# mir-group/allegro

Hardware: AMD Instinct MI355X
Metric: edge tensor-products/sec (forward+force) (higher is better)
Workload: dtype f32; 1 GPU; c4: bulk Si 23^3 cells (97 336 atoms), r_cut 5 A, l_max=2, L=2, u=64; atoms=97336, edges=2725408, parallelism=single GPU, weights=random init (reference initialisers), seed 456, workspace_bytes=21849491824

## Files before the change

### allegro_amd/_lib.py

```python
import ctypes as C
import os
from typing import Optional

import numpy as np

AA_MAX_LAYERS = 4
AA_MAX_MLP_LAYERS = 4
AA_F32, AA_F64 = 0, 1

_dp = C.POINTER(C.c_double)
_ip = C.POINTER(C.c_int32)


class TpDesc(C.Structure):
    _fields_ = [("mul", C.c_int32), ("d1", C.c_int32), ("d2", C.c_int32), ("dout", C.c_int32),
                ("num_paths", C.c_int32), ("coupling", C.c_int32), ("nnz", C.c_int32),
                ("nz_i", _ip), ("nz_j", _ip), ("nz_k", _ip), ("nz_path", _ip), ("nz_val", _dp)]


class ModelConfig(C.Structure):
    _fields_ = [("dtype", C.c_int32), ("num_types", C.c_int32), ("num_bessels", C.c_int32), ("poly_p", C.c_double),
                ("l_max", C.c_int32), ("num_layers", C.c_int32), ("num_scalar", C.c_int32), ("num_tensor", C.c_int32),
                ("embed_dim", C.c_int32), ("embed_mlp_depth", C.c_int32), ("embed_mlp_width", C.c_int32),
                ("latent_mlp_depth", C.c_int32), ("latent_mlp_width", C.c_int32),
# ... 12 lines not shown


def options_from_env() -> PlanOptions:
    env = os.environ
    flag = lambda k: int(env.get(k, "0")[:1] == "1")
    o = PlanOptions()
    o.tp_generic, o.tp_no_chain, o.tp_no_moments = flag("AA_TP_GENERIC"), flag("AA_TP_NOCHAIN"), flag("AA_TP_NOMOM")
    o.tp_no_operator, o.tp_force_operator, o.tp_operator_fused = flag("AA_TP_NOOP"), flag("AA_TP_OP"), flag("AA_OP_NOSPLIT")
    o.gemm_no_chain, o.gemm_fp32_mfma, o.gemm_valu, o.gemm_v1 = (flag("AA_GEMM_NOCHAIN"), flag("AA_GEMM_FP32_MFMA"),
                                                                 flag("AA_GEMM_VALU"), flag("AA_GEMM_V1"))
    o.gemm_lds_epilogue = int(env.get("AA_GEMM_DIRECT_EPILOGUE", "1")[:1] == "0")
    o.f64_column_loop = {"0": 1, "2": 2}.get(env.get("AA_F64_NLOOP", "1")[:1], 0)
    o.embed_no_fuse = flag("AA_EMBED_NOFUSE")
    o.fused_forward = {"0": 3, "1": 1, "2": 2, "4": 4}.get(env.get("AA_FUSED", "")[:1], 0)
    o.moments_waves_per_block = int(env.get("AA_MOM_WPB", "0") or 0)
    o.no_channel_padding = flag("AA_NO_PAD")
    o.no_slot_form = flag("AA_NO_SLOT_FORM")
    o.op_proj_gemm = {"1": 1, "0": 2}.get(env.get("AA_OP_PROJ", "")[:1], 0)
    o.op_env_vector = flag("AA_OP_ENV_VECTOR")
    o.staged_no_fold = flag("AA_STAGED_NOFOLD")
    o.op_recompute_bvecs = flag("AA_OP_RECOMPUTE_BVECS")
    o.readout_two_pass = flag("AA_READOUT_TWO_PASS")
    o.tp_prefer_moments = flag("AA_TP_PREFER_MOM")
    o.fused_narrow = {"1": 1, "2": 2, "3": 3}.get(env.get("AA_FUSED_NARROW", "")[:1], 0)
    o.chain_staged_weights = flag("AA_CHAIN_STAGED")
    o.poison_workspace = flag("AA_POISON")
    o.f64_rows = {"0": 2, "2": 1}.get(env.get("AA_F64_ROWS", "")[:1], 0)
    return o


class RawWeights(C.Structure):
    _fields_ = [("rmax_recip", _dp), ("bessel_weights", _dp), ("center_embed", _dp), ("neighbor_embed", _dp),
                ("basis_linear", _dp), ("embed_mlp", _dp * AA_MAX_MLP_LAYERS), ("env_embed_linear", _dp),
                ("first_proj", _dp), ("latent", (_dp * AA_MAX_MLP_LAYERS) * AA_MAX_LAYERS),
                ("tp_weights", _dp * AA_MAX_LAYERS), ("readout", _dp * AA_MAX_MLP_LAYERS), ("scales", _dp),
                ("shifts", _dp), ("spline_weights", _dp)]


class Graph(C.Structure):
    _fields_ = [("num_atoms", C.c_int64), ("num_edges", C.c_int64), ("center", C.c_void_p), ("nbr", C.c_void_p),
                ("rowptr", C.c_void_p), ("types", C.c_void_p), ("shift_vec", C.c_void_p),
                ("t_rowptr", C.c_void_p), ("t_perm", C.c_void_p), ("atom_begin", C.c_int64), ("atom_end", C.c_int64),
                ("max_degree", C.c_int64)]


class GemmSeg(C.Structure):
    _fields_ = [("p", C.c_void_p), ("ld", C.c_int32), ("n", C.c_int32)]
# ... 218 lines not shown
```

### allegro_amd/csrc/aa_common.h

```cpp
#pragma once
#include <type_traits>
#include <hip/hip_runtime.h>

#include <algorithm>
#include <cmath>
#include <cstdint>
#include <cstdio>
#include <cstring>
#include <string>
#include <vector>

#include "allegro_amd.h"

extern __shared__ unsigned char aa_smem[];

namespace aa {

void set_error(const std::string& msg);
int fail(int code, const std::string& msg);
int device_cu_count();

#define AA_CHECK_HIP(expr)                                                                      \
  do {                                                                                          \
    hipError_t _e = (expr);                                                                     \
// ... 538 lines not shown
  int coupling;
  float sf;
  const float* ro_w;
  float ro_factor;
  const float *scales, *shifts;
  float* vec;
  float* sh;
  float* se_h;
  float* emb;
  float* w0;
  float* lat_h0;
  float* lat_h1;
  float* ro_h;
  float* fcat;
  float *x2s0, *x2s1;
  float* atom_energy;
  int long_only;
  int32_t* status;
  int mixed;
  int skip_long, fill_done;
  float* g_fcat;
  float* g_scal1;
  int ld_gfcat;
};
size_t fused_fwd_lds_bytes(int num_types, bool teams);
enum class FusedForm { OneWave, FourWave, EightWave, EightWaveTail };
int fused_fwd_num_steps(int R);
int launch_fused_fwd(int pair, FusedForm form, const FusedFwdArgs& a, const FusedFwdArgs* wide, hipStream_t stream);
int fused_fwd8_num_steps(int R, bool tail);
size_t fused_fwd8_lds_bytes(int num_types, int waves);
int launch_fused_fwd8(int pair, FusedForm form, const FusedFwdArgs& a, hipStream_t stream);


struct EdgeGeomArgs {
  int64_t E, N;
  const int32_t *center, *nbr, *types;
  const void* pos;
  const void* shift_vec;
  int num_types, num_bessels, l_max, S0;
  double poly_p;
  const void* rmax_recip;
  const void* bessel_w;
  const void* center_embed;
  const void* neighbor_embed;
  const void* basis_w;
  int embed_kind, spline_span;
  const void* emb_tab;
  void* vec;
  void* sh;
  void* emb0;
};
template <typename T>
// ... 56 lines not shown
```

### allegro_amd/csrc/aa_fused8.hip

```cpp
#include "aa_fused_tile.h"

namespace aa {

#ifdef AA_FUSED_TIMING
__device__ unsigned long long g_fused8_ticks[32];
#define AA_TICK8(i) \
  if (blockIdx.x == gridDim.x / 2 && threadIdx.x == 0) g_fused8_ticks[i] = __builtin_readcyclecounter();
#else
#define AA_TICK8(i)
#endif

namespace {

constexpr int kLdY8 = 12;
constexpr int kOffB8 = 32 * kLdT;
constexpr int kOffY8 = kOffB8 + 9 * 64;
constexpr int kOffPark8 = kOffY8 + 32 * kLdY8;
constexpr int fused_wave_floats(int waves) { return kOffPark8 + (waves == 8 ? 2 : 1) * kTileFloats; }
static_assert(64 * kLdY8 <= 32 * kLdT, "sM must fit the patch");

template <int D>
__device__ __forceinline__ void tile_moments_half(float* sT, const float* sY, const v16f& t0, const v16f& t1, int lane, float* M) {
  const int el = lane & 31, hh = lane >> 5;
  float M0[D], M1[D];
#pragma unroll
  for (int j = 0; j < D; ++j) {
    M0[j] = 0.f;
    M1[j] = 0.f;
  }
  auto pass = [&](const v16f& t, float* Mx) {
    __builtin_amdgcn_wave_barrier();
#pragma unroll
    for (int q = 0; q < 4; ++q) *reinterpret_cast<v4f*>(sT + el * kLdT + 8 * q + 4 * hh) = v4f{t[4 * q], t[4 * q + 1], t[4 * q + 2], t[4 * q + 3]};
    __builtin_amdgcn_wave_barrier();
    const float* col = sT + (16 * hh) * kLdT + el;
    const float* yr = sY + (16 * hh) * kLdY8;
#pragma unroll 4
    for (int i = 0; i < 16; ++i) {
      const float a = col[i * kLdT];
      float y[12];
#pragma unroll
      for (int q = 0; q < (D + 3) / 4; ++q) {
        const v4f yy = *reinterpret_cast<const v4f*>(yr + i * kLdY8 + 4 * q);
#pragma unroll
        for (int c = 0; c < 4; ++c) y[4 * q + c] = yy[c];
      }
#pragma unroll
      for (int j = 0; j < D; ++j) Mx[j] += y[j] * a;
    }
    __builtin_amdgcn_wave_barrier();
  };
  pass(t0, M0);
  pass(t1, M1);
#pragma unroll
  for (int j = 0; j < D; ++j) {
    permlane32_swap(M0[j], M1[j]);
    M[j] = M0[j] + M1[j];
  }
}

template <int S, int NS, class Args, class Pipe, class F>
__device__ __forceinline__ void fused_step8(const Args& A, Pipe& p, const XSplit& x, v16f& a0, v16f& a1, F&& between) {
  pipe_issue<S, NS>(A, p);
  fused_mma_step(p.wbuf + (S & 1) * kWStep, p.lane, x, a0, a1);
  between();
  pipe_commit<S>(p);
}


__device__ __forceinline__ v16f tile_load_rows8(const float* base, unsigned ld, int lane, bool row_ok) {
  unsigned el = lane & 31;
  const unsigned hh = lane >> 5;
  opaque_vector(el);
  v16f t;
  const unsigned off = (el * ld + 4u * hh) * 4u;
#pragma unroll
  for (int q = 0; q < 4; ++q) {
    v4f v = {0.f, 0.f, 0.f, 0.f};
    if (row_ok) v = *reinterpret_cast<const v4f*>(at_bytes(base, off + 32u * q));
#pragma unroll
    for (int i = 0; i < 4; ++i) t[4 * q + i] = v[i];
// ... 38 lines not shown
    for (int i = 0; i < 4; ++i) {
      if (g < 4)
        s0[4 * q + i] += w0a[4 * q + i] * T4[i];
      else
        s1[4 * q + i] += w0b[4 * q + i] * T4[i];
    }
    if (g < 4)
      anchor(s0);
    else
      anchor(s1);
    __builtin_amdgcn_sched_barrier(0);
  }
}

struct TileIn8 {
  int beg, cnt;
  int j;
  float pi[3], pj[3], sv[3];
  int ti, tj;
};

}

constexpr int fused_fwd8_steps(int R, bool tail) { return 4 + (2 + 2 * R) + 4 + 4 + 2 + 8 + 2 + (tail ? 12 : 0); }

template <class Sig0, class Sig1, int WAVES, bool TAIL>
__global__ __launch_bounds__(64 * WAVES, 2) void fused_fwd8_kernel(FusedFwdArgs A) {
  static_assert(WAVES == 8 || WAVES == 4, "workgroup forms");
  constexpr int NT = 64 * WAVES;
  constexpr int NPARK = WAVES == 8 ? 2 : 1;
  constexpr int kWaveF = kOffPark8 + NPARK * kTileFloats;
  constexpr int D = Sig0::D2, R = Sig0::LMAX + 1;
  static_assert(Sig0::D1 == D && Sig0::DOUT == D && Sig1::D1 == D && Sig1::DOUT == 1, "standard 2-layer stack");
  static_assert(D <= 9, "l_max <= 2");
  constexpr int kPS = 4;
  constexpr int S_P0 = 0, S_L2 = kPS, S_L3 = S_L2 + 2 + 2 * R, S_P1 = S_L3 + 4, S_L6A = S_P1 + kPS, S_M = S_L6A + 2, S_L8K = S_M + 8, S_T = S_L8K + 2,
                NS = S_T + (TAIL ? 12 : 0);
  static_assert(NS % 2 == 0 && NS <= kFusedMaxSteps && NS == fused_fwd8_steps(R, TAIL), "program length");
  u32x4* wbuf = reinterpret_cast<u32x4*>(aa_smem);
  float* sRo = reinterpret_cast<float*>(wbuf + 2 * kWStep);
  float* sRm = sRo + 64;
  float* sTab = sRm + 32;
  const int ntab = A.num_types * A.num_types * 512;
  const int tid = threadIdx.x, lane = tid & 63, hh = lane >> 5, el = lane & 31;
  const int wvs = __builtin_amdgcn_readfirstlane(tid >> 6);
  float* sW = sTab + ntab + wvs * kWaveF;
  float* sBv = sW + kOffB8;
  float* sY = sW + kOffY8;
  float* sPark = sW + kOffPark8;
  for (int i = tid; i < 64; i += NT) sRo[i] = A.ro_w[i];
  if (tid < A.num_types * A.num_types) sRm[tid] = A.rmax_recip[tid];
  if (tid >= 16 && tid < 24) sRm[tid] = A.embed_kind == 0 ? A.bessel_w[tid - 16] : 0.f;
  for (int i = tid; i < ntab; i += NT) sTab[i] = A.emb_tab[i];
  std::conditional_t<WAVES == 8, FusedPipe8, FusedPipe> p;
  p.wbuf = wbuf;
  p.tid = tid;
  p.lane = lane;
  p.zero = 0;
  if constexpr (WAVES == 8) {
    p.wv = wvs;
// ... 276 lines not shown
    for (int r = 0; r < 16; ++r) {
      a60[r] = 0.f;
      a61[r] = 0.f;
      a80[r] = 0.f;
      a81[r] = 0.f;
    }
    {
      XSplit xs[2];
      v16f t;
      xsplit_from_acc(sc0, xs[0]);
      fused_step8<S_L6A + 0, NS>(A, p, xs[0], a60, a61, [&] { xsplit_from_acc(sc1, xs[1]); });
      fused_step8<S_L6A + 1, NS>(A, p, xs[1], a60, a61, [&] { xsplit_from_acc(k0, xs[0]); });
      fused_step8<S_M + 0, NS>(A, p, xs[0], a60, a61, [&] {});
      fused_step8<S_M + 1, NS>(A, p, xs[0], a80, a81, [&] { xsplit_from_acc(k1, xs[1]); });
      fused_step8<S_M + 2, NS>(A, p, xs[1], a60, a61, [&] { t = fetch_tile(sPark, lane); });
      fused_step8<S_M + 3, NS>(A, p, xs[1], a80, a81, [&] { xsplit_from_acc(t, xs[0]); });
      fused_step8<S_M + 4, NS>(A, p, xs[0], a60, a61, [&] {
        if constexpr (NPARK == 2) t = fetch_tile(sPark + kTileFloats, lane); else t = tbr;
      });
      fused_step8<S_M + 5, NS>(A, p, xs[0], a80, a81, [&] { xsplit_from_acc(t, xs[1]); });
      fused_step8<S_M + 6, NS>(A, p, xs[1], a60, a61, [&] {});
      fused_step8<S_M + 7, NS>(A, p, xs[1], a80, a81, [&] {});
      AA_TICK8(8)
      if constexpr (TAIL) {
#pragma unroll
        for (int r = 0; r < 16; ++r) {
          dk0[r] = dsilu(a60[r]);
          dk1[r] = dsilu(a61[r]);
        }
      } else {
        tile_store_rows8(sW, a60, (A.lat_h1) + row0 * 64, cnt, 64, lane);
        tile_store_rows8(sW, a61, (A.lat_h1 + 32) + row0 * 64, cnt, 64, lane);
      }
      keep_tile<true>(a60, k0);
      keep_tile<true>(a61, k1);
      xsplit_from_acc(k0, xs[0]);
      fused_step8<S_L8K + 0, NS>(A, p, xs[0], a80, a81, [&] { xsplit_from_acc(k1, xs[1]); });
      fused_step8<S_L8K + 1, NS>(A, p, xs[1], a80, a81, [&] {});
    }
    AA_TICK8(9)
    {
      if constexpr (!TAIL) {
        tile_store_rows8(sW, a80, (A.ro_h) + row0 * 64, cnt, 64, lane);
        tile_store_rows8(sW, a81, (A.ro_h + 32) + row0 * 64, cnt, 64, lane);
      }
      float part = 0.f;
#pragma unroll
      for (int q = 0; q < 4; ++q) {
        const v4f w0v = *reinterpret_cast<const v4f*>(sRo + 8 * q + 4 * hh);
        const v4f w1v = *reinterpret_cast<const v4f*>(sRo + 32 + 8 * q + 4 * hh);
#pragma unroll
        for (int i = 0; i < 4; ++i) part += silu(a80[4 * q + i]) * w0v[i] + silu(a81[4 * q + i]) * w1v[i];
      }
      float tot = row_ok ? part : 0.f;
#pragma unroll
      for (int m = 32; m >= 1; m >>= 1) tot += __shfl_xor(tot, m);
      if (atom_ok && lane == 0) {
        float en = tot * A.ro_factor;
        const int t = A.types[atom];
        if (A.scales) en *= A.scales[t];
        if (A.shifts) en += A.shifts[t];
        if (cnt < 0) en = __builtin_nanf("");
        A.atom_energy[atom] = en;
      }
    }
    if constexpr (TAIL) {
      float rofac = A.ro_factor;
      if (A.scales && atom_ok) rofac *= A.scales[A.types[atom]];
#pragma unroll
      for (int q = 0; q < 4; ++q) {
        const v4f w0v = *reinterpret_cast<const v4f*>(sRo + 8 * q + 4 * hh);
        const v4f w1v = *reinterpret_cast<const v4f*>(sRo + 32 + 8 * q + 4 * hh);
#pragma unroll
        for (int i = 0; i < 4; ++i) {
          a80[4 * q + i] = rofac * w0v[i] * dsilu(a80[4 * q + i]);
          a81[4 * q + i] = rofac * w1v[i] * dsilu(a81[4 * q + i]);
        }
      }
      XSplit xd[2], xh[2];
      xsplit_from_acc(a80, xd[0]);
      xsplit_from_acc(a81, xd[1]);
      v16f t0, t1;
      auto zero = [&] {
#pragma unroll
        for (int r = 0; r < 16; ++r) {
          t0[r] = 0.f;
          t1[r] = 0.f;
        }
      };
      zero();
      fused_step8<S_T + 0, NS>(A, p, xd[0], t0, t1, [&] {});
      fused_step8<S_T + 1, NS>(A, p, xd[1], t0, t1, [&] {});
#pragma unroll
      for (int r = 0; r < 16; ++r) {
        t0[r] *= dk0[r];
        t1[r] *= dk1[r];
      }
      xsplit_from_acc(t0, xh[0]);
      xsplit_from_acc(t1, xh[1]);
      static_for<0, 2>([&](auto pp) {
        constexpr int pr = decltype(pp)::value;
        zero();
        fused_step8<S_T + 2 + 4 * pr + 0, NS>(A, p, xd[0], t0, t1, [&] {});
        fused_step8<S_T + 2 + 4 * pr + 1, NS>(A, p, xd[1], t0, t1, [&] {});
        fused_step8<S_T + 2 + 4 * pr + 2, NS>(A, p, xh[0], t0, t1, [&] {});
        fused_step8<S_T + 2 + 4 * pr + 3, NS>(A, p, xh[1], t0, t1, [&] {});
        tile_store_rows8(sW, t0, (A.g_fcat + 64 * pr) + row0 * A.ld_gfcat, cnt, unsigned(A.ld_gfcat), lane);
        tile_store_rows8(sW, t1, (A.g_fcat + 64 * pr + 32) + row0 * A.ld_gfcat, cnt, unsigned(A.ld_gfcat), lane);
      });
      zero();
      fused_step8<S_T + 10, NS>(A, p, xh[0], t0, t1, [&] {});
      fused_step8<S_T + 11, NS>(A, p, xh[1], t0, t1, [&] {});
      tile_store_rows8(sW, t0, (A.g_scal1) + row0 * 64, cnt, 64, lane);
      tile_store_rows8(sW, t1, (A.g_scal1 + 32) + row0 * 64, cnt, 64, lane);
    }
    AA_TICK8(10)
    cur.beg = nxt.beg;
    cur.cnt = nxt.cnt;
    cur.j = nxt.j;
#pragma unroll
    for (int q = 0; q < 3; ++q) {
      cur.pi[q] = nxt.pi[q];
      cur.pj[q] = nxt.pj[q];
      cur.sv[q] = nxt.sv[q];
    }
    cur.ti = nxt.ti;
    cur.tj = nxt.tj;
    nxt.beg = beg2;
    nxt.cnt = cnt2;
    a_cur = a_nxt;
    a_nxt = a_nn;
    a_nn = a_n3;
  }
}

size_t fused_fwd8_lds_bytes(int num_types, int waves) {
  return sizeof(u32x4) * 2 * kWStep + sizeof(float) * (64 + 32 + size_t(num_types) * num_types * 512 + size_t(waves) * fused_wave_floats(waves));
}
int fused_fwd8_num_steps(int R, bool tail) { return fused_fwd8_steps(R, tail); }

int launch_fused_fwd8(int pair, FusedForm form, const FusedFwdArgs& a, hipStream_t stream) {
  if (a.atom_end <= a.atom0) return AA_OK;
  if (form == FusedForm::OneWave) return fail(AA_ERR_INVALID, "fused forward (wide): 4 or 8 waves per workgroup");
  const int waves = form == FusedForm::FourWave ? 4 : 8;
  const bool tail = form == FusedForm::EightWaveTail;
  const size_t smem = fused_fwd8_lds_bytes(a.num_types, waves);
  if (smem * (waves == 4 ? 2 : 1) > 160 * 1024) return fail(AA_ERR_INVALID, "fused forward (wide): LDS budget exceeded");
  if (!a.w0) return fail(AA_ERR_INVALID, "fused forward (wide): needs the w0 rows");
  if (tail && (!a.g_fcat || !a.g_scal1)) return fail(AA_ERR_INVALID, "fused forward (wide): the reverse tail needs its gradient outputs");
  const int cus = device_cu_count();
  if (cus < 0) return cus;
  const int64_t ngroups = (a.atom_end - a.atom0 + waves - 1) / waves;
  dim3 grid((unsigned)std::min<int64_t>(ngroups, int64_t(cus) * (waves == 4 ? 2 : 1)));
#define AA_FUSED8_LAUNCH1(S0_, S1_, W_, T_)                                                                     \
  {                                                                                                           \
    const void* fn = (const void*)fused_fwd8_kernel<cg::S0_, cg::S1_, W_, T_>;                                \
    AA_CHECK_HIP(hipFuncSetAttribute(fn, hipFuncAttributeMaxDynamicSharedMemorySize, int(smem)));             \
    hipLaunchKernelGGL((fused_fwd8_kernel<cg::S0_, cg::S1_, W_, T_>), grid, dim3(64 * W_), smem, stream, a);  \
  }
#define AA_FUSED8_LAUNCH(S0_, S1_) \
  if (tail) AA_FUSED8_LAUNCH1(S0_, S1_, 8, true) else if (waves == 8) AA_FUSED8_LAUNCH1(S0_, S1_, 8, false) else AA_FUSED8_LAUNCH1(S0_, S1_, 4, false)
  if (pair == 0) {
    AA_FUSED8_LAUNCH(Sig1, Sig0)
  } else if (pair == 1) {
    AA_FUSED8_LAUNCH(Sig5, Sig4)
  } else {
    return fail(AA_ERR_INVALID, "fused forward (wide): unsupported signature pair");
  }
#undef AA_FUSED8_LAUNCH1
#undef AA_FUSED8_LAUNCH
  AA_CHECK_HIP(hipGetLastError());
#ifdef AA_FUSED_TIMING
  {
    static int calls = 0;
    if (++calls == 8) {
      unsigned long long t[32];
      AA_CHECK_HIP(hipStreamSynchronize(stream));
      AA_CHECK_HIP(hipMemcpyFromSymbol(t, HIP_SYMBOL(g_fused8_ticks), sizeof(t)));
      static const char* nm[10] = {"geometry", "table+stores", "TPA0", "first stage", "latent0", "TPA1", "scal1", "lat1+ro merged", "lat1 epi + ro lat1", "readout epi"};
      for (int i = 0; i < 10; ++i) fprintf(stderr, "[fused8 timing] %-20s %8llu cycles\n", nm[i], t[i + 1] - t[i]);
      fprintf(stderr, "[fused8 timing] %-20s %8llu cycles\n", "total", t[10] - t[0]);
    }
  }
#endif
// ... 5 lines not shown
```

### allegro_amd/csrc/aa_model.hip

```cpp
#include <algorithm>
#include <atomic>

#include "aa_common.h"

namespace aa {
static thread_local std::string g_err;
void set_error(const std::string& msg) { g_err = msg; }
int fail(int code, const std::string& msg) {
  g_err = msg;
  return code;
}
int device_cu_count() {
  constexpr int kMaxDevices = 64;
  static std::atomic<int> cached[kMaxDevices];
  int dev = 0, n = 0;
  AA_CHECK_HIP(hipGetDevice(&dev));
  const bool slot = dev >= 0 && dev < kMaxDevices;
  if (slot && (n = cached[dev].load(std::memory_order_relaxed)) > 0) return n;
  AA_CHECK_HIP(hipDeviceGetAttribute(&n, hipDeviceAttributeMultiprocessorCount, dev));
  if (n <= 0) return fail(AA_ERR_HIP, "hipDeviceGetAttribute: the device reports no compute units");
  if (slot) cached[dev].store(n, std::memory_order_relaxed);
  return n;
}
}
// ... 1210 lines not shown
    return AA_OK;
  }
  void clear() {
    for (hipEvent_t e : events) (void)hipEventDestroy(e);
    events.clear();
    names.clear();
    bytes.clear();
    flops.clear();
  }
};

template <typename T>
struct Runner {
  const aa_model_plan* p;
  const T* wts;
  char* ws;
  Workspace w;
  int64_t E, N;
  hipStream_t stream;
  StageProfile* prof = nullptr;
  bool want_forces = false;
  bool ro_grad_done = false;
  bool fwd_b3_done = false;

  int mark(const char* name, double per_edge = 0, double per_atom = 0, double flops = 0) {
    return prof ? prof->mark(name, stream, sizeof(T) * (per_edge * double(E) + per_atom * double(N)), flops) : AA_OK;
  }
  static double seg_elems(const SegList& s) {
    double n = 0;
    for (int i = 0; i < s.count; ++i)
      if (s.s[i].p) n += s.s[i].n;
    return n;
  }
  static double gemm_row_elems(const GemmArgs& g, bool a_from_hbm) {
    double n = (a_from_hbm ? seg_elems(g.a) : 0) + seg_elems(g.c);
    for (int i = 0; i < g.c.count; ++i)
      if (g.c.s[i].p && g.c_accum[i]) n += g.c.s[i].n;
    if (g.has_z) n += seg_elems(g.z);
    if (g.has_add) n += seg_elems(g.add);
    return n;
  }

  T* buf(size_t off) const { return reinterpret_cast<T*>(ws + off); }
  const T* wt(size_t off) const { return wts + off; }

  void gemm_options(GemmArgs& g) const {
// ... 375 lines not shown
    if (!(sizeof(T) == 4 && p->pipe.fused_fwd && !p->taps && g->max_degree > 0 && g->max_degree <= kFusedMaxDegree)) return false;
    if (fused_fwd_lds_bytes(p->cfg.num_types, g->max_degree > 32) > size_t(160) * 1024) return false;
    if (g->max_degree <= 32) return true;
    const int64_t n_active = g->atom_end > g->atom_begin ? g->atom_end - g->atom_begin : g->num_atoms;
    const int64_t tiles = n_active * (g->max_degree <= 64 ? 2 : 4);
    if (p->opt.fused_forward == 2 || p->opt.fused_forward == 4) return true;
    const double fill = double(g->num_edges) / (32.0 * double(std::max<int64_t>(n_active, 1)));
    if (fill >= 0.6 && fill <= 1.15) return true;
    return tiles <= kFusedTeamTilesSmall || double(g->num_edges) >= 0.85 * 32.0 * double(tiles);
  }
  bool fold_staged() const {
    return p->pipe.chains() && p->pipe.tp_op < 0 && p->pipe.fold_embed_output && p->pipe.fold_latent_outputs && p->cfg.num_layers == 2 && !p->taps &&
           !p->opt.staged_no_fold;
  }
  bool folded_fwd(const aa_graph* g) const { return use_fused_fwd(g) || fold_staged(); }
  int fused_form(const FusedFwdArgs& a, FusedForm* form) const {
    *form = FusedForm::OneWave;
    const bool teams = a.tile_atoms != nullptr;
    if (!p->pipe.fused_wide || !a.w0 || (teams && !a.mixed)) return AA_OK;
    const int cus = device_cu_count();
    if (cus < 0) return cus;
    const int64_t n = a.atom_end - a.atom0;
    const bool tail_ok = want_forces && !teams && p->pipe.chains() && p->pipe.fold_latent_outputs && p->cfg.num_layers == 2;
    if (p->opt.fused_narrow == 2) {
      *form = tail_ok ? FusedForm::EightWaveTail : FusedForm::EightWave;
    } else if (p->opt.fused_narrow == 3) {
      *form = FusedForm::FourWave;
    } else if (n > int64_t(4) * cus) {
      *form = tail_ok && n >= int64_t(kFusedTailAtomsPerCu) * cus ? FusedForm::EightWaveTail : FusedForm::FourWave;
    }
    return AA_OK;
  }

  int forward_fused(const aa_graph* g, const void* pos, void* atom_energy) {
    const aa_model_config& c = p->cfg;
    const int S = c.num_scalar, u = c.num_tensor;
    FusedFwdArgs a{};
    a.N = N;
    a.atom0 = atom_begin(g);
    a.atom_end = atom_end(g);
    a.rowptr = g->rowptr;
    a.nbr = g->nbr;
    a.types = g->types;
    a.pos = static_cast<const float*>(pos);
    a.shift_vec = static_cast<const float*>(g->shift_vec);
    a.tile_atoms = nullptr;
    a.tile_counts = nullptr;
    a.tile_cap = 0;
    if (g->max_degree > 32) {
      a.tile_counts = reinterpret_cast<int32_t*>(buf(w.tiles));
      a.tile_atoms = a.tile_counts + 8;
      a.tile_cap = g->num_atoms;
// ... 59 lines not shown
    if (int rc = fused_form(a, &form)) return rc;
    FusedFwdArgs a8{};
    if (form != FusedForm::OneWave) {
      a8 = a;
      ns = 0;
      prog = &a8;
      auto add_step = [&](const float* Wq, int KC, int kc) {
        prog->wstep[ns][0] = Wq + (size_t(0) * KC + kc) * 64 * 24;
        prog->wstep[ns][1] = Wq + (size_t(1) * KC + kc) * 64 * 24;
        ++ns;
      };
      add_env(wf(p->o_wk0f));
      add_layer(wf(p->o_g0fq), 2, 0, 2 + 2 * p->R);
      add_layer(wf(p->latent[0].wq[0]), 4, 0, 2);
      add_env(wf(p->o_wk[1]));
      add_step(wf(p->o_lat1in_fq), 6, 4);
      add_step(wf(p->o_lat1in_fq), 6, 5);
      for (int kc : {2, 3, 0, 1}) {
        add_step(wf(p->o_lat1in_fq), 6, kc);
        add_step(wf(p->o_ro0_fq), 6, kc);
      }
      add_step(wf(p->o_ro0_fq), 6, 4);
      add_step(wf(p->o_ro0_fq), 6, 5);
      const bool tail = form == FusedForm::EightWaveTail;
      if (tail) {
        add_layer(wf(p->o_b3af_q), 2, 0, 2);
        add_layer(wf(p->pipe.fold_lat0_reverse ? p->o_b3bf_q : p->o_b3b_q), 4, 0, 4);
        add_layer(wf(p->o_b3c_q), 2, 0, 2);
        a8.g_fcat = bf(w.g_fcat);
        a8.ld_gfcat = p->SL1;
        a8.g_scal1 = bf(w.g_scal[1]);
      }
      if (ns != fused_fwd8_num_steps(p->R, tail)) return fail(AA_ERR_INVALID, "fused forward (wide): program length mismatch");
    }
    if (int rc = mark("begin")) return rc;
    if (int rc = launch_fused_fwd(p->pipe.chain_pair, form, a, form != FusedForm::OneWave ? &a8 : nullptr, stream)) return rc;
    fwd_b3_done = form == FusedForm::EightWaveTail && a.atom_end > a.atom0;
    const double per_edge = 1 + (g->shift_vec ? 3 : 0) + 3 + 4 + p->D + 5 * 64 + p->W;
    const double per_atom = 3 + 2.0 * p->D * u + 1 + 1;
    double fl = 2.0 * double(E) * (2.0 * 64 * 64 + 64.0 * p->ng0 + double(S + u) * 64 + 64.0 * S + double(2 * S + u) * 64 + 64.0 * S + 3.0 * S * 64);
    if (fwd_b3_done) {
      fl += 2.0 * double(E) * (64.0 * 64 + 128.0 * 128 + 64.0 * 64);
      return mark("fused_fwd", per_edge + 64, per_atom, fl);
    }
    return mark("fused_fwd", per_edge, per_atom, fl);
  }

  int forward(const aa_graph* g, const void* pos, void* atom_energy) {
    const aa_model_config& c = p->cfg;
    const int S = c.num_scalar, u = c.num_tensor, L = c.num_layers, W = p->W, SL1 = p->SL1;
    if (use_fused_fwd(g)) return forward_fused(g, pos, atom_energy);
    if (int rc = mark("begin")) return rc;
    const double idx2 = 8.0 / sizeof(T);
    if (int rc = launch_edge_prologue<T>(geom(g, pos), stream)) return rc;
    if (int rc = mark("edge_prologue", idx2 + 6 + (g->shift_vec ? 3 : 0) + 4 + p->D + c.embed_dim)) return rc;
    const SegList none{0, {}};
    const bool slot = use_slot();
    const bool fstaged = fold_staged();
    if (p->pipe.chains()) {
      ChainArgs ca{};
      ca.nlayers = 3;
      SegList in{1, {seg(buf(w.emb0), c.embed_dim, c.embed_dim)}};
      SegList c0{1, {seg(buf(w.se_h[0]), 64, 64)}};
      SegList c1{1, {seg(buf(w.emb), S, S)}};
      SegList c2{2, {seg(buf(w.fcat), SL1, S), seg(buf(w.w0), W, W)}};
// ... 302 lines not shown
            return rc;
          a = cs;
        }
      } else {
        r.g_h = buf(w.g_fcat);
        if (int rc = launch_readout_backward<T>(r, stream)) return rc;
        if (int rc = mark("readout_backward", 2.0 * (c.readout_mlp_depth > 0 ? c.readout_mlp_width : SL1))) return rc;
      }
    }
    const double sfac = 1.0 / std::sqrt(c.avg_num_neighbors);
    for (int l = L - 1; l >= 0; --l) {
      if (p->pipe.chains() && l == L - 1) {
      } else if (p->pipe.chains()) {
        ChainArgs ca{};
        ca.nlayers = 2;
        SegList in{1, {seg(buf(w.g_fcat) + S * (l + 1), SL1, S)}};
        SegList cn{1, {seg(nullptr, 64, 64)}};
        SegList zz{1, {seg(buf(w.lat_h[l][0]), 64, 64)}};
        SegList ad{1, {seg(buf(w.g_aenv), 64, 64)}};
        SegList c1{2, {seg(buf(w.g_fcat), SL1, S * (l + 1)), seg(buf(w.g_scal[l]), u, u)}};
        int acc1[3] = {1, 0, 0};
        ca.L[0] = chain_layer(E, in, 0, wt(p->latent[l].wtq[1]), S, 64, cn, nullptr, &zz, &ad, 0, 0, 0);
        ca.L[1] = chain_layer(E, none, 0, wt(p->latent[l].wtq[0]), 64, S * (l + 1) + u, c1, acc1, nullptr, nullptr, 1, -1, 0);
        if (p->pipe.fold_lat0_reverse && L == 2 && l == 0) {
          ca.nlayers = 1;
          ca.L[0] = chain_layer(E, in, 0, wt(p->latent[l].wtq[0]), 64, S * (l + 1) + u, c1, acc1, nullptr, nullptr, 0, -1, 0);
          ca.L[0].a_mode = 2;
          ca.L[0].a2_add = buf(w.g_aenv);
          ca.L[0].ld_a2add = 64;
          ca.L[0].a2_z = buf(w.lat_h[l][0]);
          ca.L[0].ld_a2z = 64;
          if (sizeof(T) == 4 && S == 64 && u == 64 && !p->opt.chain_staged_weights) {
            ChainB2Args b2{};
            b2.M = E;
            b2.a = reinterpret_cast<const float*>(buf(w.g_fcat)) + S * (l + 1);
            b2.lda = SL1;
            b2.add = reinterpret_cast<const float*>(buf(w.g_aenv));
            b2.ldadd = 64;
            b2.z = reinterpret_cast<const float*>(buf(w.lat_h[l][0]));
            b2.ldz = 64;
            b2.Wq = wt(p->latent[l].wtq[0]);
            b2.c0 = reinterpret_cast<float*>(buf(w.g_fcat));
            b2.ldc0 = SL1;
            b2.c1 = reinterpret_cast<float*>(buf(w.g_scal[l]));
            b2.ldc1 = u;
            if (int rc = launch_chain_b2_resident(b2, stream)) return rc;
// ... 6 lines not shown
      } else {
      SegList go;
      go.count = (l < L - 1 && !p->pipe.env_moments()) ? 2 : 1;
      go.s[0] = seg(buf(w.g_fcat) + S * (l + 1), SL1, S);
      if (l < L - 1 && !p->pipe.env_moments()) go.s[1] = seg(buf(w.g_envw), W, W);
      SegList aenv{1, {seg(p->pipe.env_moments() ? buf(w.g_aenv) : nullptr, c.latent_mlp_width, c.latent_mlp_width)}};
      const SegList* addp = (p->pipe.env_moments() && l < L - 1) ? &aenv : nullptr;
      SegList gi{2, {seg(buf(w.g_fcat), SL1, S * (l + 1)), seg(buf(w.g_scal[l]), u, u)}};
      int acc[3] = {1, 0, 0};
      if (int rc = mlp_bwd(p->latent[l], c.latent_mlp_depth + 1, go, w.lat_h[l], w.g_lat_h, gi, acc, 1, addp)) return rc;
      }
      if (p->pipe.tp_op >= 0) {
        if (int rc = run_op_bwd(g, l)) return rc;
        continue;
      }
      if (p->pipe.env_moments()) {
        TpMomArgs m = mom_args(g);
        m.c.gscal0 = buf(w.g_scal[0]);
        m.c.gscal1 = buf(w.g_scal[1]);
        m.c.g_w0 = buf(w.g_w0);
        m.c.gsh_x1 = buf(w.g_sh);
        m.c.gsh_env = buf(w.g_sh) + size_t(l + 1) * size_t(E) * p->D;
        m.g_a = buf(w.g_aenv);
        if (l == 1) {
          m.ld_ga = c.latent_mlp_width;
          if (int rc = launch_tp_mom_bwd_last<T>(p->pipe.chain_pair, m, stream)) return rc;
          if (int rc = mark("tp_mom_bwd_last", p->D + W + u + 2 * m.ka1 + p->D, double(p->D) * u)) return rc;
        } else {
          m.ld_ga = S;
          if (p->pipe.fold_embed_output && folded_fwd(g)) m.wt0 = wt(p->o_wt0f);
          if (int rc = launch_tp_mom_bwd_first<T>(p->pipe.chain_pair, m, stream)) return rc;
          if (int rc = mark("tp_mom_bwd_first", p->D + 2 * W + 2 * u + 2 * m.ka0 + 2 * p->D, 2.0 * p->D * u)) return rc;
        }
        continue;
      }
      if (p->pipe.chain_pair >= 0) {
        TpChainArgs a = chain_args(g);
        a.gscal0 = buf(w.g_scal[0]);
        a.gscal1 = buf(w.g_scal[1]);
        a.g_w0 = buf(w.g_w0);
        a.g_wenv = buf(w.g_envw);
        a.gsh_x1 = buf(w.g_sh);
        a.gsh_env = buf(w.g_sh) + size_t(l + 1) * size_t(E) * p->D;
        if (l == 1) {
          if (int rc = launch_tp_chain_bwd_last<T>(p->pipe.chain_pair, a, stream)) return rc;
          if (int rc = mark("tp_chain_bwd_last", 3 * W + 2 * p->D + u, 2.0 * p->D * u)) return rc;
        } else {
// ... 281 lines not shown
```

Baseline: 625.5 million edge-TP/s.

## Fuse layer-0 reverse stages into an eight-wave deep tail of the fused forward kernel

Adds an EightWaveDeepTail form to the fused forward kernel. It also does the last-layer moment backward (projecting gradient moments through the tensor-product weights, producing env spherical-harmonic gradients) and the layer-0 latent backward GEMMs into g_fcat and g_scal0. It keeps the layer-1 gradient tile parked in LDS instead of writing and re-reading it. The host then skips the separate tp_mom_bwd_last and layer-0 chain launches. This removes intermediate global-memory traffic and kernel launches, at the cost of a longer per-workgroup program, more register and LDS pressure, and extra weight-streaming steps.

After: 674.7 million edge-TP/s, median of 6. 1.08x the previous value.

```diff
diff --git a/allegro_amd/_lib.py b/allegro_amd/_lib.py
--- a/allegro_amd/_lib.py
+++ b/allegro_amd/_lib.py
@@ -58,7 +58,7 @@
     o.op_recompute_bvecs = flag("AA_OP_RECOMPUTE_BVECS")
     o.readout_two_pass = flag("AA_READOUT_TWO_PASS")
     o.tp_prefer_moments = flag("AA_TP_PREFER_MOM")
-    o.fused_narrow = {"1": 1, "2": 2, "3": 3}.get(env.get("AA_FUSED_NARROW", "")[:1], 0)
+    o.fused_narrow = {"1": 1, "2": 2, "3": 3, "4": 4}.get(env.get("AA_FUSED_NARROW", "")[:1], 0)
     o.chain_staged_weights = flag("AA_CHAIN_STAGED")
     o.poison_workspace = flag("AA_POISON")
     o.f64_rows = {"0": 2, "2": 1}.get(env.get("AA_F64_ROWS", "")[:1], 0)
diff --git a/allegro_amd/csrc/aa_common.h b/allegro_amd/csrc/aa_common.h
--- a/allegro_amd/csrc/aa_common.h
+++ b/allegro_amd/csrc/aa_common.h
@@ -584,12 +584,14 @@
   float* g_fcat;
   float* g_scal1;
   int ld_gfcat;
+  float* g_scal0;
+  float* gsh_env1;
 };
 size_t fused_fwd_lds_bytes(int num_types, bool teams);
-enum class FusedForm { OneWave, FourWave, EightWave, EightWaveTail };
+enum class FusedForm { OneWave, FourWave, EightWave, EightWaveTail, EightWaveDeepTail };
 int fused_fwd_num_steps(int R);
 int launch_fused_fwd(int pair, FusedForm form, const FusedFwdArgs& a, const FusedFwdArgs* wide, hipStream_t stream);
-int fused_fwd8_num_steps(int R, bool tail);
+int fused_fwd8_num_steps(int R, int tail);
 size_t fused_fwd8_lds_bytes(int num_types, int waves);
 int launch_fused_fwd8(int pair, FusedForm form, const FusedFwdArgs& a, hipStream_t stream);
 
diff --git a/allegro_amd/csrc/aa_fused8.hip b/allegro_amd/csrc/aa_fused8.hip
--- a/allegro_amd/csrc/aa_fused8.hip
+++ b/allegro_amd/csrc/aa_fused8.hip
@@ -19,12 +19,12 @@
 constexpr int fused_wave_floats(int waves) { return kOffPark8 + (waves == 8 ? 2 : 1) * kTileFloats; }
 static_assert(64 * kLdY8 <= 32 * kLdT, "sM must fit the patch");
 
-template <int D>
+template <int D, int J0 = 0, int NJ = D>
 __device__ __forceinline__ void tile_moments_half(float* sT, const float* sY, const v16f& t0, const v16f& t1, int lane, float* M) {
   const int el = lane & 31, hh = lane >> 5;
-  float M0[D], M1[D];
-#pragma unroll
-  for (int j = 0; j < D; ++j) {
+  float M0[NJ], M1[NJ];
+#pragma unroll
+  for (int j = 0; j < NJ; ++j) {
     M0[j] = 0.f;
     M1[j] = 0.f;
   }
@@ -40,23 +40,70 @@
       const float a = col[i * kLdT];
       float y[12];
 #pragma unroll
-      for (int q = 0; q < (D + 3) / 4; ++q) {
+      for (int q = J0 / 4; q < (J0 + NJ + 3) / 4; ++q) {
         const v4f yy = *reinterpret_cast<const v4f*>(yr + i * kLdY8 + 4 * q);
 #pragma unroll
         for (int c = 0; c < 4; ++c) y[4 * q + c] = yy[c];
       }
 #pragma unroll
-      for (int j = 0; j < D; ++j) Mx[j] += y[j] * a;
+      for (int j = 0; j < NJ; ++j) Mx[j] += y[J0 + j] * a;
     }
     __builtin_amdgcn_wave_barrier();
   };
   pass(t0, M0);
   pass(t1, M1);
 #pragma unroll
-  for (int j = 0; j < D; ++j) {
+  for (int j = 0; j < NJ; ++j) {
     permlane32_swap(M0[j], M1[j]);
     M[j] = M0[j] + M1[j];
   }
+}
+
+template <int S0, int NS, int D, int R, int LDY, class Args, class Pipe>
+__device__ __forceinline__ void project_moments_t(const Args& A, Pipe& p, float* sM, const float* g, float sf, float* out) {
+  const int lane = p.lane;
+#pragma unroll
+  for (int q = 0; q < (D + 3) / 4; ++q) {
+    v4f mm;
+#pragma unroll
+    for (int i = 0; i < 4; ++i) mm[i] = 4 * q + i < D ? g[4 * q + i] : 0.f;
+    *reinterpret_cast<v4f*>(sM + lane * LDY + 4 * q) = mm;
+  }
+  __builtin_amdgcn_wave_barrier();
+#pragma unroll
+  for (int j = 0; j < D; ++j) out[j] = 0.f;
+  static_for<0, 4>([&](auto cc) {
+    constexpr int c = decltype(cc)::value;
+    constexpr int S = S0 + c;
+    constexpr int row0 = 48 * c < 64 * R - 48 ? 48 * c : 64 * R - 48;
+    constexpr int lo = 48 * c, hi = 48 * (c + 1) < 64 * R ? 48 * (c + 1) : 64 * R;
+    pipe_issue<S, NS>(A, p);
+    const float* wf = reinterpret_cast<const float*>(p.wbuf + (S & 1) * kWStep) + lane;
+    static_for<0, 24>([&](auto pp) {
+      static_for<0, 2>([&](auto hh2) {
+        constexpr int L = lo + 2 * decltype(pp)::value + decltype(hh2)::value;
+        if constexpr (L < hi) {
+          constexpr int r = L / 64, ch = L % 64, j0 = r * r, nj = 2 * r + 1;
+          const float w = wf[(L - row0) * 64];
+          float m[12];
+#pragma unroll
+          for (int q = j0 / 4; q < (j0 + nj + 3) / 4; ++q) {
+            const v4f mv = *reinterpret_cast<const v4f*>(sM + ch * LDY + 4 * q);
+#pragma unroll
+            for (int i = 0; i < 4; ++i) m[4 * q + i] = mv[i];
+          }
+#pragma unroll
+          for (int j = j0; j < j0 + nj; ++j) out[j] += m[j] * w;
+        }
+      });
+#pragma unroll
+      for (int j = 0; j < D; ++j) anchor(out[j]);
+      __builtin_amdgcn_sched_barrier(0);
+    });
+    pipe_commit<S>(p);
+  });
+#pragma unroll
+  for (int j = 0; j < D; ++j) out[j] *= sf;
 }
 
 template <int S, int NS, class Args, class Pipe, class F>
@@ -141,11 +188,12 @@
 
 }
 
-constexpr int fused_fwd8_steps(int R, bool tail) { return 4 + (2 + 2 * R) + 4 + 4 + 2 + 8 + 2 + (tail ? 12 : 0); }
-
-template <class Sig0, class Sig1, int WAVES, bool TAIL>
+constexpr int fused_fwd8_steps(int R, int tail) { return 4 + (2 + 2 * R) + 4 + 4 + 2 + 8 + 2 + (tail == 2 ? 20 : tail == 1 ? 12 : 0); }
+
+template <class Sig0, class Sig1, int WAVES, int TAIL>
 __global__ __launch_bounds__(64 * WAVES, 2) void fused_fwd8_kernel(FusedFwdArgs A) {
   static_assert(WAVES == 8 || WAVES == 4, "workgroup forms");
+  static_assert(TAIL >= 0 && TAIL <= 2 && (TAIL == 0 || WAVES == 8), "the tails exist for the eight-wave form");
   constexpr int NT = 64 * WAVES;
   constexpr int NPARK = WAVES == 8 ? 2 : 1;
   constexpr int kWaveF = kOffPark8 + NPARK * kTileFloats;
@@ -154,7 +202,8 @@
   static_assert(D <= 9, "l_max <= 2");
   constexpr int kPS = 4;
   constexpr int S_P0 = 0, S_L2 = kPS, S_L3 = S_L2 + 2 + 2 * R, S_P1 = S_L3 + 4, S_L6A = S_P1 + kPS, S_M = S_L6A + 2, S_L8K = S_M + 8, S_T = S_L8K + 2,
-                NS = S_T + (TAIL ? 12 : 0);
+                S_Q = S_T + 12, S_B2 = S_Q + kPS, NS = S_T + (TAIL == 2 ? 12 + kPS + 4 : TAIL == 1 ? 12 : 0);
+  constexpr bool DEEP = TAIL == 2;
   static_assert(NS % 2 == 0 && NS <= kFusedMaxSteps && NS == fused_fwd8_steps(R, TAIL), "program length");
   u32x4* wbuf = reinterpret_cast<u32x4*>(aa_smem);
   float* sRo = reinterpret_cast<float*>(wbuf + 2 * kWStep);
@@ -477,7 +526,7 @@
       fused_step8<S_M + 6, NS>(A, p, xs[1], a60, a61, [&] {});
       fused_step8<S_M + 7, NS>(A, p, xs[1], a80, a81, [&] {});
       AA_TICK8(8)
-      if constexpr (TAIL) {
+      if constexpr (TAIL != 0) {
 #pragma unroll
         for (int r = 0; r < 16; ++r) {
           dk0[r] = dsilu(a60[r]);
@@ -495,7 +544,7 @@
     }
     AA_TICK8(9)
     {
-      if constexpr (!TAIL) {
+      if constexpr (TAIL == 0) {
         tile_store_rows8(sW, a80, (A.ro_h) + row0 * 64, cnt, 64, lane);
         tile_store_rows8(sW, a81, (A.ro_h + 32) + row0 * 64, cnt, 64, lane);
       }
@@ -519,7 +568,7 @@
         A.atom_energy[atom] = en;
       }
     }
-    if constexpr (TAIL) {
+    if constexpr (TAIL != 0) {
       float rofac = A.ro_factor;
       if (A.scales && atom_ok) rofac *= A.scales[A.types[atom]];
 #pragma unroll
@@ -560,14 +609,132 @@
         fused_step8<S_T + 2 + 4 * pr + 1, NS>(A, p, xd[1], t0, t1, [&] {});
         fused_step8<S_T + 2 + 4 * pr + 2, NS>(A, p, xh[0], t0, t1, [&] {});
         fused_step8<S_T + 2 + 4 * pr + 3, NS>(A, p, xh[1], t0, t1, [&] {});
-        tile_store_rows8(sW, t0, (A.g_fcat + 64 * pr) + row0 * A.ld_gfcat, cnt, unsigned(A.ld_gfcat), lane);
-        tile_store_rows8(sW, t1, (A.g_fcat + 64 * pr + 32) + row0 * A.ld_gfcat, cnt, unsigned(A.ld_gfcat), lane);
+        if constexpr (DEEP && pr == 1) {
+          park_tile(sPark, t0, lane);
+          park_tile(sPark + kTileFloats, t1, lane);
+        } else {
+          tile_store_rows8(sW, t0, (A.g_fcat + 64 * pr) + row0 * A.ld_gfcat, cnt, unsigned(A.ld_gfcat), lane);
+          tile_store_rows8(sW, t1, (A.g_fcat + 64 * pr + 32) + row0 * A.ld_gfcat, cnt, unsigned(A.ld_gfcat), lane);
+        }
       });
       zero();
       fused_step8<S_T + 10, NS>(A, p, xh[0], t0, t1, [&] {});
       fused_step8<S_T + 11, NS>(A, p, xh[1], t0, t1, [&] {});
       tile_store_rows8(sW, t0, (A.g_scal1) + row0 * 64, cnt, 64, lane);
       tile_store_rows8(sW, t1, (A.g_scal1 + 32) + row0 * 64, cnt, 64, lane);
+      if constexpr (DEEP) {
+        float GM[D];
+        {
+          float q1[D];
+          v16f wa = tile_load_rows8(A.w0 + row0 * (64 * R), 64 * R, lane, row_ok), wb = tile_load_rows8(A.w0 + row0 * (64 * R) + 32, 64 * R, lane, row_ok);
+          static_for<0, R>([&](auto rr) {
+            constexpr int r = decltype(rr)::value;
+            v16f na = wa, nb = wb;
+            if constexpr (r + 1 < R) {
+              na = tile_load_rows8(A.w0 + row0 * (64 * R) + (r + 1) * 64, 64 * R, lane, row_ok);
+              nb = tile_load_rows8(A.w0 + row0 * (64 * R) + (r + 1) * 64 + 32, 64 * R, lane, row_ok);
+            }
+#pragma unroll
+            for (int i = 0; i < 16; ++i) {
+              wa[i] *= t0[i];
+              wb[i] *= t1[i];
+            }
+            tile_moments_half<D, r * r, 2 * r + 1>(sW, sY, wa, wb, lane, q1 + r * r);
+            wa = na;
+            wb = nb;
+          });
+          float wp0[Sig0::P], wp1[Sig1::P];
+#pragma unroll
+          for (int q = 0; q < Sig0::P; ++q) wp0[q] = load_pw(A.tpw0, Sig0::P, q);
+#pragma unroll
+          for (int q = 0; q < Sig1::P; ++q) wp1[q] = load_pw(A.tpw1, Sig1::P, q);
+          float x2s0b[D], tq[D], g2[D], one[1] = {1.f};
+#pragma unroll
+          for (int j = 0; j < D; ++j) x2s0b[j] = atom_ok ? *at_bytes(A.x2s0 + (atom * D + j) * 64, 4u * unsigned(lane)) : 0.f;
+          Sig0::template fwd<float>(q1, x2s0b, wp0, tq);
+          Sig1::template bx2<float>(one, tq, wp1, g2);
+          project_moments_t<S_Q, NS, D, R, kLdY8>(A, p, sW, g2, A.sf, GM);
+        }
+        __builtin_amdgcn_wave_barrier();
+#pragma unroll
+        for (int a = 0; a < D; ++a) sBv[a * 64 + lane] = GM[a];
+        __builtin_amdgcn_wave_barrier();
+        v16f h0a = tile_load_rows8(A.lat_h0 + row0 * 64, 64, lane, row_ok), h0b = tile_load_rows8(A.lat_h0 + row0 * 64 + 32, 64, lane, row_ok);
+        {
+          float Yv[D], gy[D];
+          load_Y(Yv);
+#pragma unroll
+          for (int a = 0; a < D; ++a) gy[a] = 0.f;
+          const float* bb = sBv + 4 * hh;
+#pragma unroll
+          for (int g = 0; g < 8; ++g) {
+            const int q = g & 3;
+            v4f T4 = {0.f, 0.f, 0.f, 0.f}, av;
+#pragma unroll
+            for (int i = 0; i < 4; ++i) av[i] = silu(g < 4 ? h0a[4 * q + i] : h0b[4 * q + i]);
+#pragma unroll
+            for (int a = 0; a < D; ++a) {
+              const v4f b = *reinterpret_cast<const v4f*>(bb + a * 64 + 32 * (g >> 2) + 8 * q);
+#pragma unroll
+              for (int i = 0; i < 4; ++i) {
+                T4[i] += Yv[a] * b[i];
+                gy[a] += av[i] * b[i];
+              }
+            }
+#pragma unroll
+            for (int i = 0; i < 4; ++i) {
+              if (g < 4)
+                t0[4 * q + i] = T4[i];
+              else
+                t1[4 * q + i] = T4[i];
+            }
+            if (g < 4)
+              anchor(t0);
+            else
+              anchor(t1);
+#pragma unroll
+            for (int a = 0; a < D; ++a) anchor(gy[a]);
+            __builtin_amdgcn_sched_barrier(0);
+          }
+#pragma unroll
+          for (int a = 0; a < D; ++a) gy[a] += __shfl_xor(gy[a], 32);
+          if (row_ok && hh == 0) {
+            float* gb = A.gsh_env1 + row0 * D;
+#pragma unroll
+            for (int m = 0; m < D; ++m) *at_bytes(gb, 4u * (unsigned(el) * D + m)) = gy[m];
+          }
+        }
+        XSplit xo[2];
+        {
+          v16f da = fetch_tile(sPark, lane);
+#pragma unroll
+          for (int r = 0; r < 16; ++r) t0[r] = (da[r] + t0[r]) * dsilu(h0a[r]);
+          da = fetch_tile(sPark + kTileFloats, lane);
+#pragma unroll
+          for (int r = 0; r < 16; ++r) t1[r] = (da[r] + t1[r]) * dsilu(h0b[r]);
+          xsplit_from_acc(t0, xo[0]);
+          xsplit_from_acc(t1, xo[1]);
+        }
+        zero();
+        fused_step8<S_B2 + 0, NS>(A, p, xo[0], t0, t1, [&] {});
+        fused_step8<S_B2 + 1, NS>(A, p, xo[1], t0, t1, [&] {});
+        {
+          const v16f oa = tile_load_rows8(A.g_fcat + row0 * A.ld_gfcat, unsigned(A.ld_gfcat), lane, row_ok);
+          const v16f ob = tile_load_rows8(A.g_fcat + row0 * A.ld_gfcat + 32, unsigned(A.ld_gfcat), lane, row_ok);
+#pragma unroll
+          for (int r = 0; r < 16; ++r) {
+            t0[r] += oa[r];
+            t1[r] += ob[r];
+          }
+        }
+        tile_store_rows8(sW, t0, (A.g_fcat) + row0 * A.ld_gfcat, cnt, unsigned(A.ld_gfcat), lane);
+        tile_store_rows8(sW, t1, (A.g_fcat + 32) + row0 * A.ld_gfcat, cnt, unsigned(A.ld_gfcat), lane);
+        zero();
+        fused_step8<S_B2 + 2, NS>(A, p, xo[0], t0, t1, [&] {});
+        fused_step8<S_B2 + 3, NS>(A, p, xo[1], t0, t1, [&] {});
+        tile_store_rows8(sW, t0, (A.g_scal0) + row0 * 64, cnt, 64, lane);
+        tile_store_rows8(sW, t1, (A.g_scal0 + 32) + row0 * 64, cnt, 64, lane);
+      }
     }
     AA_TICK8(10)
     cur.beg = nxt.beg;
@@ -592,17 +759,18 @@
 size_t fused_fwd8_lds_bytes(int num_types, int waves) {
   return sizeof(u32x4) * 2 * kWStep + sizeof(float) * (64 + 32 + size_t(num_types) * num_types * 512 + size_t(waves) * fused_wave_floats(waves));
 }
-int fused_fwd8_num_steps(int R, bool tail) { return fused_fwd8_steps(R, tail); }
+int fused_fwd8_num_steps(int R, int tail) { return fused_fwd8_steps(R, tail); }
 
 int launch_fused_fwd8(int pair, FusedForm form, const FusedFwdArgs& a, hipStream_t stream) {
   if (a.atom_end <= a.atom0) return AA_OK;
   if (form == FusedForm::OneWave) return fail(AA_ERR_INVALID, "fused forward (wide): 4 or 8 waves per workgroup");
   const int waves = form == FusedForm::FourWave ? 4 : 8;
-  const bool tail = form == FusedForm::EightWaveTail;
+  const int tail = form == FusedForm::EightWaveDeepTail ? 2 : form == FusedForm::EightWaveTail ? 1 : 0;
   const size_t smem = fused_fwd8_lds_bytes(a.num_types, waves);
   if (smem * (waves == 4 ? 2 : 1) > 160 * 1024) return fail(AA_ERR_INVALID, "fused forward (wide): LDS budget exceeded");
   if (!a.w0) return fail(AA_ERR_INVALID, "fused forward (wide): needs the w0 rows");
   if (tail && (!a.g_fcat || !a.g_scal1)) return fail(AA_ERR_INVALID, "fused forward (wide): the reverse tail needs its gradient outputs");
+  if (tail == 2 && (!a.g_scal0 || !a.gsh_env1)) return fail(AA_ERR_INVALID, "fused forward (wide): the deep tail needs its gradient outputs");
   const int cus = device_cu_count();
   if (cus < 0) return cus;
   const int64_t ngroups = (a.atom_end - a.atom0 + waves - 1) / waves;
@@ -614,7 +782,7 @@
     hipLaunchKernelGGL((fused_fwd8_kernel<cg::S0_, cg::S1_, W_, T_>), grid, dim3(64 * W_), smem, stream, a);  \
   }
 #define AA_FUSED8_LAUNCH(S0_, S1_) \
-  if (tail) AA_FUSED8_LAUNCH1(S0_, S1_, 8, true) else if (waves == 8) AA_FUSED8_LAUNCH1(S0_, S1_, 8, false) else AA_FUSED8_LAUNCH1(S0_, S1_, 4, false)
+  if (tail == 2) AA_FUSED8_LAUNCH1(S0_, S1_, 8, 2) else if (tail == 1) AA_FUSED8_LAUNCH1(S0_, S1_, 8, 1) else if (waves == 8) AA_FUSED8_LAUNCH1(S0_, S1_, 8, 0) else AA_FUSED8_LAUNCH1(S0_, S1_, 4, 0)
   if (pair == 0) {
     AA_FUSED8_LAUNCH(Sig1, Sig0)
   } else if (pair == 1) {
diff --git a/allegro_amd/csrc/aa_model.hip b/allegro_amd/csrc/aa_model.hip
--- a/allegro_amd/csrc/aa_model.hip
+++ b/allegro_amd/csrc/aa_model.hip
@@ -1256,6 +1256,7 @@
   bool want_forces = false;
   bool ro_grad_done = false;
   bool fwd_b3_done = false;
+  bool fwd_b2_done = false;
 
   int mark(const char* name, double per_edge = 0, double per_atom = 0, double flops = 0) {
     return prof ? prof->mark(name, stream, sizeof(T) * (per_edge * double(E) + per_atom * double(N)), flops) : AA_OK;
@@ -1677,12 +1678,15 @@
     if (cus < 0) return cus;
     const int64_t n = a.atom_end - a.atom0;
     const bool tail_ok = want_forces && !teams && p->pipe.chains() && p->pipe.fold_latent_outputs && p->cfg.num_layers == 2;
-    if (p->opt.fused_narrow == 2) {
-      *form = tail_ok ? FusedForm::EightWaveTail : FusedForm::EightWave;
+    const bool deep_ok = tail_ok && p->pipe.fold_lat0_reverse && p->pipe.env_moments() && sizeof(T) == 4 && p->cfg.num_scalar == 64 &&
+                         p->cfg.num_tensor == 64 && p->cfg.latent_mlp_width == 64 && p->opt.fused_narrow != 4;
+    const FusedForm tail_form = deep_ok ? FusedForm::EightWaveDeepTail : FusedForm::EightWaveTail;
+    if (p->opt.fused_narrow == 2 || p->opt.fused_narrow == 4) {
+      *form = tail_ok ? tail_form : FusedForm::EightWave;
     } else if (p->opt.fused_narrow == 3) {
       *form = FusedForm::FourWave;
     } else if (n > int64_t(4) * cus) {
-      *form = tail_ok && n >= int64_t(kFusedTailAtomsPerCu) * cus ? FusedForm::EightWaveTail : FusedForm::FourWave;
+      *form = tail_ok && n >= int64_t(kFusedTailAtomsPerCu) * cus ? tail_form : FusedForm::FourWave;
     }
     return AA_OK;
   }
@@ -1788,7 +1792,8 @@
       }
       add_step(wf(p->o_ro0_fq), 6, 4);
       add_step(wf(p->o_ro0_fq), 6, 5);
-      const bool tail = form == FusedForm::EightWaveTail;
+      const bool deep = form == FusedForm::EightWaveDeepTail;
+      const bool tail = deep || form == FusedForm::EightWaveTail;
       if (tail) {
         add_layer(wf(p->o_b3af_q), 2, 0, 2);
         add_layer(wf(p->pipe.fold_lat0_reverse ? p->o_b3bf_q : p->o_b3b_q), 4, 0, 4);
@@ -1797,16 +1802,32 @@
         a8.ld_gfcat = p->SL1;
         a8.g_scal1 = bf(w.g_scal[1]);
       }
-      if (ns != fused_fwd8_num_steps(p->R, tail)) return fail(AA_ERR_INVALID, "fused forward (wide): program length mismatch");
+      if (deep) {
+        for (int cblk = 0; cblk < 4; ++cblk) {
+          const int row0 = std::min(48 * cblk, 64 * p->R - 48);
+          prog->wstep[ns][0] = wf(p->o_wt[1]) + size_t(row0) * 64;
+          prog->wstep[ns][1] = wf(p->o_wt[1]) + size_t(row0) * 64 + 1536;
+          ++ns;
+        }
+        add_layer(wf(p->latent[0].wtq[0]), 2, 0, 4);
+        a8.g_scal0 = bf(w.g_scal[0]);
+        a8.gsh_env1 = bf(w.g_sh) + size_t(2) * size_t(E) * p->D;
+      }
+      if (ns != fused_fwd8_num_steps(p->R, deep ? 2 : tail ? 1 : 0)) return fail(AA_ERR_INVALID, "fused forward (wide): program length mismatch");
     }
     if (int rc = mark("begin")) return rc;
     if (int rc = launch_fused_fwd(p->pipe.chain_pair, form, a, form != FusedForm::OneWave ? &a8 : nullptr, stream)) return rc;
-    fwd_b3_done = form == FusedForm::EightWaveTail && a.atom_end > a.atom0;
+    fwd_b2_done = form == FusedForm::EightWaveDeepTail && a.atom_end > a.atom0;
+    fwd_b3_done = (fwd_b2_done || form == FusedForm::EightWaveTail) && a.atom_end > a.atom0;
     const double per_edge = 1 + (g->shift_vec ? 3 : 0) + 3 + 4 + p->D + 5 * 64 + p->W;
     const double per_atom = 3 + 2.0 * p->D * u + 1 + 1;
     double fl = 2.0 * double(E) * (2.0 * 64 * 64 + 64.0 * p->ng0 + double(S + u) * 64 + 64.0 * S + double(2 * S + u) * 64 + 64.0 * S + 3.0 * S * 64);
     if (fwd_b3_done) {
       fl += 2.0 * double(E) * (64.0 * 64 + 128.0 * 128 + 64.0 * 64);
+      if (fwd_b2_done) {
+        fl += 2.0 * double(E) * 64.0 * 128;
+        return mark("fused_fwd", per_edge + 64 + 64 + p->D, per_atom, fl);
+      }
       return mark("fused_fwd", per_edge + 64, per_atom, fl);
     }
     return mark("fused_fwd", per_edge, per_atom, fl);
@@ -2155,6 +2176,7 @@
         int acc1[3] = {1, 0, 0};
         ca.L[0] = chain_layer(E, in, 0, wt(p->latent[l].wtq[1]), S, 64, cn, nullptr, &zz, &ad, 0, 0, 0);
         ca.L[1] = chain_layer(E, none, 0, wt(p->latent[l].wtq[0]), 64, S * (l + 1) + u, c1, acc1, nullptr, nullptr, 1, -1, 0);
+        if (fwd_b2_done && l == 0) goto b2_done;
         if (p->pipe.fold_lat0_reverse && L == 2 && l == 0) {
           ca.nlayers = 1;
           ca.L[0] = chain_layer(E, in, 0, wt(p->latent[l].wtq[0]), 64, S * (l + 1) + u, c1, acc1, nullptr, nullptr, 0, -1, 0);
@@ -2207,7 +2229,8 @@
         m.c.gsh_x1 = buf(w.g_sh);
         m.c.gsh_env = buf(w.g_sh) + size_t(l + 1) * size_t(E) * p->D;
         m.g_a = buf(w.g_aenv);
-        if (l == 1) {
+        if (l == 1 && fwd_b2_done) {
+        } else if (l == 1) {
           m.ld_ga = c.latent_mlp_width;
           if (int rc = launch_tp_mom_bwd_last<T>(p->pipe.chain_pair, m, stream)) return rc;
           if (int rc = mark("tp_mom_bwd_last", p->D + W + u + 2 * m.ka1 + p->D, double(p->D) * u)) return rc;
```
